# QZ1-boy/CDFO

Hardware: NVIDIA B200
Metric: HR frames/sec, 1080p x4 LD-QP37 (higher is better)
Workload: dtype bf16

## Files before the change

cdfo_b200/csrc/lra.cu:

```cuda
#include <cuda.h>
#include <cstring>

#include "cdfo_common.cuh"
#include "sm100_ptx.cuh"

namespace cdfo {

__device__ __forceinline__ float warp_max(float v) {
#pragma unroll
  for (int o = 16; o > 0; o >>= 1) v = fmaxf(v, __shfl_xor_sync(0xffffffffu, v, o));
  return v;
}
__device__ __forceinline__ float warp_sum(float v) {
#pragma unroll
  for (int o = 16; o > 0; o >>= 1) v += __shfl_xor_sync(0xffffffffu, v, o);
  return v;
}

__global__ void lra_mask_kernel(const float *__restrict__ u, const float *__restrict__ vmax, const float *__restrict__ qv,
                                uint8_t *__restrict__ midx, float *__restrict__ qsel, int HW) {
  __shared__ float vm[64];
  const int b = blockIdx.y;
  if (threadIdx.x < 64) vm[threadIdx.x] = vmax[b * 64 + threadIdx.x];
  __syncthreads();
  const int p = blockIdx.x * blockDim.x + threadIdx.x;
  if (p >= HW) return;
  const float *up = u + (size_t)b * 64 * HW + p;
  float lmax = -INFINITY, second_sum = 0.f;
  int cmax = 0;
  float l[64];
#pragma unroll
  for (int c = 0; c < 64; ++c) {
    const float g = -logf(-logf(up[(size_t)c * HW]));
    l[c] = vm[c] + g;
    if (l[c] > lmax) { lmax = l[c]; cmax = c; }
  }
#pragma unroll
  for (int c = 0; c < 64; ++c) second_sum += expf(l[c] - lmax);
  const bool on = (1.0f / second_sum) >= 0.5f;
  midx[(size_t)b * HW + p] = on ? (uint8_t)cmax : (uint8_t)255;
  qsel[(size_t)b * HW + p] = on ? qv[((size_t)b * 128 + cmax) * HW + p] : 0.f;
}

constexpr int kLd = 68;
__device__ __forceinline__ uint32_t to_tf32(float x) {
  uint32_t r;
  asm("cvt.rna.tf32.f32 %0, %1;" : "=r"(r) : "f"(x));
  return r;
}
__device__ __forceinline__ void mma_tf32(float (&d)[4], const uint32_t (&a)[4], uint32_t b0, uint32_t b1) {
  asm volatile("mma.sync.aligned.m16n8k8.row.col.f32.tf32.tf32.f32 {%0, %1, %2, %3}, {%4, %5, %6, %7}, {%8, %9}, {%0, %1, %2, %3};"
               : "+f"(d[0]), "+f"(d[1]), "+f"(d[2]), "+f"(d[3])
               : "r"(a[0]), "r"(a[1]), "r"(a[2]), "r"(a[3]), "r"(b0), "r"(b1));
}


__device__ __forceinline__ void flash_tile_block(float (&sc)[8][4], float (&m_run)[2], float (&l_run)[2], float (&o)[8][4],
                                                 const uint32_t *__restrict__ Vu, int key0, int n_keys, int g, int tq) {
  float mx[2] = {-INFINITY, -INFINITY};
#pragma unroll
  for (int n = 0; n < 8; ++n) {
    const int key = key0 + 8 * n + 2 * tq;
    if (key >= n_keys) { sc[n][0] = -INFINITY; sc[n][2] = -INFINITY; }
    if (key + 1 >= n_keys) { sc[n][1] = -INFINITY; sc[n][3] = -INFINITY; }
    mx[0] = fmaxf(mx[0], fmaxf(sc[n][0], sc[n][1]));
    mx[1] = fmaxf(mx[1], fmaxf(sc[n][2], sc[n][3]));
  }
  float scale[2];
#pragma unroll
  for (int r = 0; r < 2; ++r) {
    mx[r] = fmaxf(mx[r], __shfl_xor_sync(0xffffffffu, mx[r], 1));
    mx[r] = fmaxf(mx[r], __shfl_xor_sync(0xffffffffu, mx[r], 2));
    const float m_new = fmaxf(m_run[r], mx[r]);
    scale[r] = expf(m_run[r] - m_new);
    m_run[r] = m_new;
    l_run[r] *= scale[r];
  }
#pragma unroll
  for (int n = 0; n < 8; ++n) {
    sc[n][0] = expf(sc[n][0] - m_run[0]); sc[n][1] = expf(sc[n][1] - m_run[0]);
    sc[n][2] = expf(sc[n][2] - m_run[1]); sc[n][3] = expf(sc[n][3] - m_run[1]);
    l_run[0] += sc[n][0] + sc[n][1];
    l_run[1] += sc[n][2] + sc[n][3];
    o[n][0] *= scale[0]; o[n][1] *= scale[0]; o[n][2] *= scale[1]; o[n][3] *= scale[1];
  }
#pragma unroll
  for (int s = 0; s < 8; ++s) {
    const uint32_t ap[4] = {to_tf32(sc[s][0]), to_tf32(sc[s][2]), to_tf32(sc[s][1]), to_tf32(sc[s][3])};
    const uint32_t *vr = Vu + (key0 + 8 * s + 2 * tq) * kLd + g;
#pragma unroll
    for (int n = 0; n < 8; ++n) mma_tf32(o[n], ap, vr[8 * n], vr[kLd + 8 * n]);
  }
}

constexpr int kRowWarps = 9, kRowThreads = kRowWarps * 32;
constexpr int kRowPiece = 64;
constexpr int kRowRawBytes = 2 * 64 * kRowPiece * 4 + 64;
template <bool TMA>
__global__ void __launch_bounds__(kRowThreads, 1) lra_row_kernel(const __grid_constant__ CUtensorMap qvmap, const float *__restrict__ qv,
                                                                const uint8_t *__restrict__ midx, const float *__restrict__ qsel,
                                                                float *__restrict__ vrow_t, LraTables t, int H, int W) {
  extern __shared__ __align__(1024) float sm_all[];
  float *sm = TMA ? sm_all + kRowRawBytes / 4 : sm_all;
  const int b = blockIdx.y, h = blockIdx.x;
  const int HW = H * W;
  const int Wk = (W + 63) & ~63;
  float *vr = sm;
  float *Rs = vr + Wk * kLd;
  float *sw = Rs + 4096;
  float *e0 = sw + Wk;
  float *qs = e0 + Wk;
  float *n0 = qs + Wk;
  float *red = n0 + 64;
  int *cs = reinterpret_cast<int *>(red + kRowThreads);
  int *mlist = cs + Wk;
  __shared__ int mcount;
  __shared__ float m0_s, d0_s;
  const int tid = threadIdx.x, lane = tid & 31, warp = tid >> 5, g = lane >> 2, tq = lane & 3;
  float kw[9];
#pragma unroll
  for (int i = 0; i < 9; ++i) kw[i] = t.kw[i];
  for (int e = tid; e < 4096; e += kRowThreads) Rs[e] = t.r[e];

  if (TMA) {
    float *raw = sm_all;
    uint64_t *bars = reinterpret_cast<uint64_t *>(sm_all + 2 * 64 * kRowPiece);
    const uint32_t bar0 = ptx::smem_u32(bars);
    if (tid == 0) {
      ptx::mbar_init(bar0, 1);
      ptx::mbar_init(bar0 + 8, 1);
      ptx::mbar_init(bar0 + 16, 8);
      ptx::mbar_init(bar0 + 24, 8);
      ptx::fence_mbar_init();
    }
    __syncthreads();
    const int n_pieces = Wk / kRowPiece;
    if (warp == 8) {
      if (lane == 0) {
        for (int pc = 0; pc < n_pieces; ++pc) {
          const int st = pc & 1;
          ptx::mbar_wait_parked(bar0 + 16 + 8 * st, ((pc >> 1) & 1) ^ 1);
          ptx::mbar_arrive_expect_tx(bar0 + 8 * st, 64 * kRowPiece * 4);
          ptx::tma_load_3d(ptx::smem_u32(raw) + st * 64 * kRowPiece * 4, &qvmap, bar0 + 8 * st, pc * kRowPiece, h, b * 128 + 64);
        }
      }
    } else {
      const int px = tid & 63, c0 = (tid >> 6) * 16;
      for (int pc = 0; pc < n_pieces; ++pc) {
        const int st = pc & 1, w = pc * kRowPiece + px;
        ptx::mbar_wait_parked(bar0 + 8 * st, (pc >> 1) & 1);
        const float *rp = raw + st * 64 * kRowPiece + px;
        float win[24];
#pragma unroll
        for (int i = 0; i < 24; ++i) {
          const int c = c0 - 4 + i;
          win[i] = (c >= 0 && c < 64) ? rp[c * kRowPiece] : 0.f;
        }
        __syncwarp();
        if (lane == 0) ptx::mbar_arrive(bar0 + 16 + 8 * st);
        float *row = vr + w * kLd + c0;
#pragma unroll
        for (int c4 = 0; c4 < 4; ++c4) {
          float o[4];
#pragma unroll
          for (int j = 0; j < 4; ++j) {
            float acc = t.beta;
#pragma unroll
            for (int i = 0; i < 9; ++i) acc = fmaf(kw[i], win[4 * c4 + j + i], acc);
            o[j] = w < W ? acc : 0.f;
          }
          *reinterpret_cast<float4 *>(row + 4 * c4) = make_float4(o[0], o[1], o[2], o[3]);
        }
      }
    }
  } else {
  const float *vbase = qv + ((size_t)b * 128 + 64) * HW + (size_t)h * W;
  for (int e = tid; e < 64 * Wk; e += kRowThreads) {
    const int c = e / Wk, w = e - c * Wk;
    const bool ok = w < W;
// ... 14 lines not shown
    for (int c4 = 0; c4 < 16; ++c4) {
      const float4 v = *reinterpret_cast<const float4 *>(row + 4 * c4);
      win[4 + 4 * c4] = v.x; win[5 + 4 * c4] = v.y; win[6 + 4 * c4] = v.z; win[7 + 4 * c4] = v.w;
    }
#pragma unroll
    for (int c4 = 0; c4 < 16; ++c4) {
      float o[4];
#pragma unroll
      for (int j = 0; j < 4; ++j) {
        float acc = t.beta;
#pragma unroll
        for (int i = 0; i < 9; ++i) acc = fmaf(kw[i], win[4 * c4 + j + i], acc);
        o[j] = acc;
      }
      *reinterpret_cast<float4 *>(row + 4 * c4) = make_float4(o[0], o[1], o[2], o[3]);
    }
  }
  }
  if (tid == 0) mcount = 0;
  __syncthreads();
  for (int w = tid; w < Wk; w += kRowThreads) {
    int c = 255;
    float q = 0.f;
    if (w < W) {
      c = midx[(size_t)b * HW + h * W + w];
      q = qsel[(size_t)b * HW + h * W + w];
    }
    const bool on = c != 255;
    cs[w] = on ? c : -1;
    qs[w] = q;
    sw[w] = on ? t.beta * q * t.k1[c] : 0.f;
    if (on) mlist[atomicAdd(&mcount, 1)] = w;
  }
  __syncthreads();
  float m = -INFINITY;
  for (int w = tid; w < W; w += kRowThreads) m = fmaxf(m, sw[w]);
  m = warp_max(m);
  if (lane == 0) red[warp] = m;
  __syncthreads();
  if (tid == 0) {
    float mm = red[0];
    for (int i = 1; i < kRowWarps; ++i) mm = fmaxf(mm, red[i]);
    m0_s = mm;
  }
  __syncthreads();
  const float m0 = m0_s;
  float d = 0.f;
  for (int w = tid; w < W; w += kRowThreads) {
    const float e = expf(sw[w] - m0);
    e0[w] = e;
    d += e;
  }
  d = warp_sum(d);
  __syncthreads();
  if (lane == 0) red[warp] = d;
  __syncthreads();
  if (tid == 0) {
    float dd = 0.f;
    for (int i = 0; i < kRowWarps; ++i) dd += red[i];
    d0_s = dd;
  }
  {
    const int c = tid & 63, part = tid >> 6;
    float acc = 0.f;
    if (part < 4)
      for (int w = part; w < W; w += 4) acc = fmaf(e0[w], vr[w * kLd + c], acc);
    __syncthreads();
    red[tid] = acc;
    __syncthreads();
    if (tid < 64) n0[tid] = (red[tid] + red[tid + 64] + red[tid + 128] + red[tid + 192]) / d0_s;
  }
  __syncthreads();
  for (int e = tid; e < W * 64; e += kRowThreads) {
    const int w = e >> 6, c = e & 63;
    if (cs[w] < 0) vrow_t[(((size_t)b * W + w) * H + h) * 64 + c] = n0[c];
  }
  for (int e = tid; e < Wk * 64; e += kRowThreads) {
    float *p = vr + (e >> 6) * kLd + (e & 63);
    *p = __uint_as_float(to_tf32(*p));
  }
  __syncthreads();
  const int nm = mcount;
  const uint32_t *Vu = reinterpret_cast<const uint32_t *>(vr);
  for (int q0 = warp * 16; q0 < nm; q0 += kRowWarps * 16) {
    int wq[2], c1[2];
    float q1[2];
#pragma unroll
    for (int r = 0; r < 2; ++r) {
      const int qi = q0 + g + 8 * r;
      wq[r] = qi < nm ? mlist[qi] : -1;
      c1[r] = wq[r] >= 0 ? cs[wq[r]] : 0;
      q1[r] = wq[r] >= 0 ? qs[wq[r]] : 0.f;
    }
    float o[8][4];
#pragma unroll
    for (int n = 0; n < 8; ++n)
#pragma unroll
      for (int i = 0; i < 4; ++i) o[n][i] = 0.f;
    float m_run[2] = {-INFINITY, -INFINITY}, l_run[2] = {0.f, 0.f};
    for (int key0 = 0; key0 < Wk; key0 += 64) {
      float sc[8][4];
#pragma unroll
      for (int n = 0; n < 8; ++n) {
        const int k = key0 + 8 * n + 2 * tq;
        const float2 s2 = *reinterpret_cast<const float2 *>(sw + k), q2 = *reinterpret_cast<const float2 *>(qs + k);
        const int2 c2 = *reinterpret_cast<const int2 *>(cs + k);
#pragma unroll
        for (int r = 0; r < 2; ++r) {
          sc[n][2 * r] = c2.x >= 0 ? fmaf(q1[r] * q2.x, Rs[c1[r] * 64 + c2.x], s2.x) : s2.x;
          sc[n][2 * r + 1] = c2.y >= 0 ? fmaf(q1[r] * q2.y, Rs[c1[r] * 64 + c2.y], s2.y) : s2.y;
        }
      }
      flash_tile_block(sc, m_run, l_run, o, Vu, key0, W, g, tq);
    }
#pragma unroll
    for (int r = 0; r < 2; ++r) {
      l_run[r] += __shfl_xor_sync(0xffffffffu, l_run[r], 1);
      l_run[r] += __shfl_xor_sync(0xffffffffu, l_run[r], 2);
    }
#pragma unroll
    for (int r = 0; r < 2; ++r) {
      if (wq[r] < 0) continue;
      const float inv = 1.f / l_run[r];
      float *dst = vrow_t + (((size_t)b * W + wq[r]) * H + h) * 64 + 2 * tq;
#pragma unroll
      for (int n = 0; n < 8; ++n) *reinterpret_cast<float2 *>(dst + 8 * n) = make_float2(o[n][2 * r] * inv, o[n][2 * r + 1] * inv);
    }
  }
}


template <typename LoadKV, typename Store>
__device__ __forceinline__ void flash_block_fp32_kptr(const float *Qs, const float *const *Kptr, const float *Vs, float *Ps,
                                                      int n_keys, LoadKV key_chunk, Store store) {
  const int tid = threadIdx.x, ty = tid >> 4, tx = tid & 15;
  float m_run[4], l_run[4], o[4][4];
#pragma unroll
  for (int i = 0; i < 4; ++i) {
    m_run[i] = -INFINITY;
    l_run[i] = 0.f;
#pragma unroll
    for (int c = 0; c < 4; ++c) o[i][c] = 0.f;
  }
  const int n_chunks = (n_keys + 63) >> 6;
  for (int kb = 0; kb < n_chunks; ++kb) {
    key_chunk(kb);
    const float *Ks = *Kptr;
    float sacc[4][4];
#pragma unroll
    for (int i = 0; i < 4; ++i)
#pragma unroll
      for (int j = 0; j < 4; ++j) sacc[i][j] = 0.f;
#pragma unroll 4
    for (int k = 0; k < 64; k += 4) {
      float4 a[4], bq[4];
#pragma unroll
      for (int i = 0; i < 4; ++i) a[i] = *reinterpret_cast<const float4 *>(Qs + (ty + 16 * i) * kLd + k);
#pragma unroll
      for (int j = 0; j < 4; ++j) bq[j] = *reinterpret_cast<const float4 *>(Ks + (tx + 16 * j) * kLd + k);
#pragma unroll
      for (int i = 0; i < 4; ++i)
#pragma unroll
        for (int j = 0; j < 4; ++j) {
          sacc[i][j] = fmaf(a[i].x, bq[j].x, sacc[i][j]);
          sacc[i][j] = fmaf(a[i].y, bq[j].y, sacc[i][j]);
          sacc[i][j] = fmaf(a[i].z, bq[j].z, sacc[i][j]);
          sacc[i][j] = fmaf(a[i].w, bq[j].w, sacc[i][j]);
        }
    }
#pragma unroll
    for (int i = 0; i < 4; ++i) {
      float mx = -INFINITY;
#pragma unroll
      for (int j = 0; j < 4; ++j) {
        if (kb * 64 + tx + 16 * j >= n_keys) sacc[i][j] = -INFINITY;
        mx = fmaxf(mx, sacc[i][j]);
      }
#pragma unroll
      for (int off = 8; off > 0; off >>= 1) mx = fmaxf(mx, __shfl_xor_sync(0xffffffffu, mx, off));
      const float m_new = fmaxf(m_run[i], mx);
      const float scale = expf(m_run[i] - m_new);
      m_run[i] = m_new;
      float ps = 0.f;
#pragma unroll
      for (int j = 0; j < 4; ++j) {
        const float pv = expf(sacc[i][j] - m_new);
        Ps[(ty + 16 * i) * kLd + tx + 16 * j] = pv;
        ps += pv;
      }
      l_run[i] = l_run[i] * scale + ps;
#pragma unroll
      for (int c = 0; c < 4; ++c) o[i][c] *= scale;
    }
    __syncthreads();
#pragma unroll 4
    for (int j = 0; j < 64; j += 4) {
      float4 pr[4], vv[4];
#pragma unroll
      for (int i = 0; i < 4; ++i) pr[i] = *reinterpret_cast<const float4 *>(Ps + (ty + 16 * i) * kLd + j);
#pragma unroll
      for (int jj = 0; jj < 4; ++jj) vv[jj] = *reinterpret_cast<const float4 *>(Vs + (j + jj) * kLd + 4 * tx);
#pragma unroll
      for (int i = 0; i < 4; ++i) {
        const float pe[4] = {pr[i].x, pr[i].y, pr[i].z, pr[i].w};
#pragma unroll
        for (int jj = 0; jj < 4; ++jj) {
          o[i][0] = fmaf(pe[jj], vv[jj].x, o[i][0]);
          o[i][1] = fmaf(pe[jj], vv[jj].y, o[i][1]);
          o[i][2] = fmaf(pe[jj], vv[jj].z, o[i][2]);
// ... 367 lines not shown
    }
  }
  float mx[2] = {-INFINITY, -INFINITY}, sum[2] = {0.f, 0.f};
#pragma unroll
  for (int n = 0; n < 8; ++n) {
    mx[0] = fmaxf(mx[0], fmaxf(sc[n][0], sc[n][1]));
    mx[1] = fmaxf(mx[1], fmaxf(sc[n][2], sc[n][3]));
  }
#pragma unroll
  for (int r = 0; r < 2; ++r) {
    mx[r] = fmaxf(mx[r], __shfl_xor_sync(0xffffffffu, mx[r], 1));
    mx[r] = fmaxf(mx[r], __shfl_xor_sync(0xffffffffu, mx[r], 2));
  }
#pragma unroll
  for (int n = 0; n < 8; ++n) {
    sc[n][0] = expf(sc[n][0] - mx[0]); sc[n][1] = expf(sc[n][1] - mx[0]);
    sc[n][2] = expf(sc[n][2] - mx[1]); sc[n][3] = expf(sc[n][3] - mx[1]);
    sum[0] += sc[n][0] + sc[n][1];
    sum[1] += sc[n][2] + sc[n][3];
  }
  float o[8][4];
#pragma unroll
  for (int n = 0; n < 8; ++n)
#pragma unroll
    for (int i = 0; i < 4; ++i) o[n][i] = 0.f;
#pragma unroll
  for (int s = 0; s < 4; ++s) {
    uint32_t ap[4], apl[4];
#pragma unroll
    for (int i = 0; i < 4; ++i) {
      const float p0 = sc[2 * s + (i >> 1)][2 * (i & 1)], p1 = sc[2 * s + (i >> 1)][2 * (i & 1) + 1];
      const float h0 = __bfloat162float(__float2bfloat16_rn(p0)), h1 = __bfloat162float(__float2bfloat16_rn(p1));
      ap[i] = pack_bf16x2(h0, h1);
      apl[i] = pack_bf16x2(p0 - h0, p1 - h1);
    }
    const uint32_t *vr = Vt + g * kWinLd + 8 * s + tq, *vl = Vl + g * kWinLd + 8 * s + tq;
#pragma unroll
    for (int n = 0; n < 8; ++n) {
      const uint32_t b0 = vr[8 * n * kWinLd], b1 = vr[8 * n * kWinLd + 4];
      mma_bf16(o[n], apl, b0, b1);
      mma_bf16(o[n], ap, vl[8 * n * kWinLd], vl[8 * n * kWinLd + 4]);
      mma_bf16(o[n], ap, b0, b1);
    }
  }
#pragma unroll
  for (int r = 0; r < 2; ++r) {
    sum[r] += __shfl_xor_sync(0xffffffffu, sum[r], 1);
    sum[r] += __shfl_xor_sync(0xffffffffu, sum[r], 2);
  }
  const float inv0 = 1.f / sum[0], inv1 = 1.f / sum[1];
  const int t0 = q0r + g, t1 = t0 + 8;
  float *d0 = loc_out + (((size_t)b * H + wy * 8 + (t0 >> 3)) * W + wx * 8 + (t0 & 7)) * 64 + 2 * tq;
  float *d1 = loc_out + (((size_t)b * H + wy * 8 + (t1 >> 3)) * W + wx * 8 + (t1 & 7)) * 64 + 2 * tq;
#pragma unroll
  for (int n = 0; n < 8; ++n) {
    *reinterpret_cast<float2 *>(d0 + 8 * n) = make_float2(o[n][0] * inv0, o[n][1] * inv0);
    *reinterpret_cast<float2 *>(d1 + 8 * n) = make_float2(o[n][2] * inv1, o[n][3] * inv1);
  }
}

}

using namespace cdfo;

typedef CUresult (*LraEncodeTiledFn)(CUtensorMap *, CUtensorMapDataType, cuuint32_t, void *, const cuuint64_t *, const cuuint64_t *,
                                     const cuuint32_t *, const cuuint32_t *, CUtensorMapInterleave, CUtensorMapSwizzle,
                                     CUtensorMapL2promotion, CUtensorMapFloatOOBfill);
static LraEncodeTiledFn lra_encode_tiled_fn() {
  static LraEncodeTiledFn fn = nullptr;
  if (!fn) {
    void *ptr = nullptr;
    cudaDriverEntryPointQueryResult q;
    if (cudaGetDriverEntryPoint("cuTensorMapEncodeTiled", &ptr, cudaEnableDefault, &q) == cudaSuccess && q == cudaDriverEntryPointSuccess)
      fn = reinterpret_cast<LraEncodeTiledFn>(ptr);
  }
  return fn;
}

static bool g_lra_row_tma = true;
extern "C" int cdfo_lra_set_row_tma(int on) {
  g_lra_row_tma = on != 0;
  return CDFO_OK;
}
static bool g_lra_col_tf32 = false;
static bool g_lra_col_tc = true;
static bool g_lra_win_tc = true;
extern "C" int cdfo_lra_set_col_precision(int tf32) {
  g_lra_col_tf32 = tf32 != 0;
  return CDFO_OK;
}
extern "C" int cdfo_lra_set_col_tcgen05(int on) {
  g_lra_col_tc = on != 0;
  return CDFO_OK;
}
extern "C" int cdfo_lra_set_win_tensor_core(int on) {
  g_lra_win_tc = on != 0;
  return CDFO_OK;
}

extern "C" size_t cdfo_lra_workspace_bytes(int B, int H, int W) {
  const size_t P = (size_t)B * H * W;
  return P * (1 + 4) + 3 * P * 64 * 4 + 256;
}

static int lra_run(const float *qv, const float *u, const float *vmax, const float *x, const float *x2, const float *tables,
                   float beta, float bh, const float *fuse_w, const float *fuse_b, float *out, void *out_c8, int out_channels,
                   int channel0, void *workspace, int B, int H, int W, void *stream);

extern "C" int cdfo_lra_fwd(const float *qv, const float *u, const float *vmax, const float *x, const float *x2, const float *tables,
                            float beta, float bh, const float *fuse_w, const float *fuse_b, float *out, void *workspace, int B,
                            int H, int W, void *stream) {
  return lra_run(qv, u, vmax, x, x2, tables, beta, bh, fuse_w, fuse_b, out, nullptr, 0, 0, workspace, B, H, W, stream);
}

extern "C" int cdfo_lra_c8_fwd(const float *qv, const float *u, const float *vmax, const float *x, const float *x2, const float *tables,
                               float beta, float bh, const float *fuse_w, const float *fuse_b, void *out_c8, int out_channels,
                               int channel0, void *workspace, int B, int H, int W, void *stream) {
  CDFO_REQUIRE(out_c8 && ((uintptr_t)out_c8 & 15) == 0, CDFO_ERR_NULL, "cdfo_lra_c8_fwd: out_c8 must be a 16-byte aligned pointer");
  CDFO_REQUIRE(out_channels % 8 == 0 && channel0 % 8 == 0 && channel0 >= 0 && channel0 + 64 <= out_channels, CDFO_ERR_SHAPE,
               "cdfo_lra_c8_fwd: channels [%d, %d) do not fit %d output channels (multiples of 8)", channel0, channel0 + 64, out_channels);
  return lra_run(qv, u, vmax, x, x2, tables, beta, bh, fuse_w, fuse_b, nullptr, out_c8, out_channels, channel0, workspace, B, H, W, stream);
}

static int lra_run(const float *qv, const float *u, const float *vmax, const float *x, const float *x2, const float *tables,
                   float beta, float bh, const float *fuse_w, const float *fuse_b, float *out, void *out_c8, int out_channels,
                   int channel0, void *workspace, int B, int H, int W, void *stream) {
  CDFO_REQUIRE(qv && u && vmax && x && tables && fuse_w && fuse_b && (out || out_c8) && workspace, CDFO_ERR_NULL, "cdfo_lra_fwd: NULL pointer");
  CDFO_REQUIRE(B > 0 && B <= 65535 && H > 0 && W > 0 && H % 8 == 0 && W % 8 == 0, CDFO_ERR_SHAPE,
               "cdfo_lra_fwd: H and W must be multiples of the window size 8 (got %d x %d)", H, W);
  cudaStream_t s = (cudaStream_t)stream;
  const size_t P = (size_t)B * H * W;
  const int HW = H * W;
  uint8_t *ws = (uint8_t *)workspace;
  float *qsel = (float *)ws;
  float *vrow_t = qsel + P;
  float *long_out = vrow_t + P * 64;
  float *loc_out = long_out + P * 64;
  uint8_t *midx = (uint8_t *)(loc_out + P * 64);
  LraTables t{tables, tables + 9, tables + 18, tables + 82, beta, bh};

  lra_mask_kernel<<<dim3(ceil_div(HW, 128), B), 128, 0, s>>>(u, vmax, qv, midx, qsel, HW);

  const int Wk = (W + 63) & ~63;
  const size_t row_smem = ((size_t)Wk * kLd + 4096 + 3 * (size_t)Wk + 64 + kRowThreads + 2 * (size_t)Wk) * 4;
  const int Hk = (H + 63) & ~63;
  const size_t col_v = (size_t)Hk * kLd > (size_t)(H + 8) * 64 ? (size_t)Hk * kLd : (size_t)(H + 8) * 64;
  const size_t col_smem = ((size_t)Hk * kLd + col_v) * 4;
  const size_t win_smem = (size_t)3 * 64 * kLd * 4;
  const int kDynMax = 224 * 1024;
  CDFO_REQUIRE(row_smem <= (size_t)kDynMax && col_smem <= (size_t)kDynMax, CDFO_ERR_UNSUPPORTED,
               "cdfo_lra_fwd: frame %d x %d exceeds the shared-memory row/column buffers (W <= 704, H <= 384)", H, W);
  static bool attr = false;
  if (!attr) {
    cudaError_t e1 = cudaFuncSetAttribute(lra_row_kernel<false>, cudaFuncAttributeMaxDynamicSharedMemorySize, kDynMax);
    if (e1 == cudaSuccess) e1 = cudaFuncSetAttribute(lra_row_kernel<true>, cudaFuncAttributeMaxDynamicSharedMemorySize, kDynMax);
    cudaError_t e2 = cudaFuncSetAttribute(lra_col_kernel, cudaFuncAttributeMaxDynamicSharedMemorySize, kDynMax);
    if (e2 == cudaSuccess) e2 = cudaFuncSetAttribute(lra_col_bf16_kernel, cudaFuncAttributeMaxDynamicSharedMemorySize, kDynMax);
    cudaError_t e3 = cudaFuncSetAttribute(lra_win_kernel, cudaFuncAttributeMaxDynamicSharedMemorySize, (int)win_smem);
    if (e1 != cudaSuccess || e2 != cudaSuccess || e3 != cudaSuccess)
      return fail(CDFO_ERR_CUDA, "cdfo_lra_fwd: cudaFuncSetAttribute failed: %s", cudaGetErrorString(e1 != cudaSuccess ? e1 : (e2 != cudaSuccess ? e2 : e3)));
    attr = true;
  }
  {
    CUtensorMap qm;
    memset(&qm, 0, sizeof(qm));
    bool row_tma = g_lra_row_tma && W % 4 == 0 && ((uintptr_t)qv & 15) == 0 && row_smem + kRowRawBytes <= (size_t)kDynMax;
    if (row_tma) {
      static LraEncodeTiledFn enc = lra_encode_tiled_fn();
      if (enc) {
        const cuuint64_t gdim[3] = {(cuuint64_t)W, (cuuint64_t)H, (cuuint64_t)B * 128};
        const cuuint64_t gstr[2] = {(cuuint64_t)W * 4, (cuuint64_t)H * W * 4};
        const cuuint32_t box[3] = {kRowPiece, 1, 64};
        const cuuint32_t estr[3] = {1, 1, 1};
        CUresult cr = enc(&qm, CU_TENSOR_MAP_DATA_TYPE_FLOAT32, 3, const_cast<float *>(qv), gdim, gstr, box, estr, CU_TENSOR_MAP_INTERLEAVE_NONE,
                          CU_TENSOR_MAP_SWIZZLE_NONE, CU_TENSOR_MAP_L2_PROMOTION_L2_128B, CU_TENSOR_MAP_FLOAT_OOB_FILL_NONE);
        CDFO_REQUIRE(cr == CUDA_SUCCESS, CDFO_ERR_CUDA, "cuTensorMapEncodeTiled(qv rows) failed with CUresult %d", (int)cr);
      } else {
        row_tma = false;
      }
    }
    if (row_tma) lra_row_kernel<true><<<dim3(H, B), kRowThreads, row_smem + kRowRawBytes, s>>>(qm, qv, midx, qsel, vrow_t, t, H, W);
    else lra_row_kernel<false><<<dim3(H, B), kRowThreads, row_smem, s>>>(qm, qv, midx, qsel, vrow_t, t, H, W);
  }
  int col_done = 0;
  if (!g_lra_col_tf32 && g_lra_col_tc) {
    col_done = lra_col_sm100_launch(vrow_t, midx, qsel, long_out, t, B, H, W, s);
    if (col_done < 0) return col_done;
  }
  if (col_done) {
  } else if (g_lra_col_tf32) {
    lra_col_kernel<<<dim3(W, B), kColThreads, col_smem, s>>>(vrow_t, midx, qsel, long_out, t, H, W);
  } else {
    const size_t col16_smem = ((size_t)Hk * kQw + 64 * ((size_t)Hk / 2 + 4) + 2 * (size_t)(H + 8) + 16) * 4;
    lra_col_bf16_kernel<<<dim3(W, B), kColThreads, col16_smem, s>>>(vrow_t, midx, qsel, long_out, t, H, W);
  }
  if (g_lra_win_tc) lra_win_tc_kernel<<<dim3(W / 8, H / 8, B), kWinTcThreads, 0, s>>>(qv, midx, loc_out, H, W);
  else lra_win_kernel<<<dim3(W / 8, H / 8, B), kWinThreads, win_smem, s>>>(qv, midx, loc_out, H, W);
  if (int rc = check_launch("cdfo_lra_fwd")) return rc;
  return pointwise_conv(long_out, loc_out, fuse_w, fuse_b, x, x2, out, B, 128, 64, HW, 0, 1, s, out_c8, out_channels, channel0);
}
```

include/cdfo_b200.h:

```cpp
#ifndef CDFO_B200_H_
#define CDFO_B200_H_

#include <stddef.h>
#include <stdint.h>

#ifdef __cplusplus
extern "C" {
#endif

typedef enum cdfo_status {
  CDFO_OK = 0,
  CDFO_ERR_SHAPE = -1,
  CDFO_ERR_NULL = -2,
  CDFO_ERR_CUDA = -3,
  CDFO_ERR_UNSUPPORTED = -4,
  CDFO_ERR_NO_DEVICE = -5
} cdfo_status;

typedef enum cdfo_dtype { CDFO_F32 = 0, CDFO_F16 = 1, CDFO_BF16 = 2 } cdfo_dtype;
#define CDFO_FIELDS_F16X4 16

const char *cdfo_last_error(void);
int cdfo_version(void);
int cdfo_device_ok(int dev);
// ... 2 lines not shown
                 const void *bias, void *y, int B, int C, int H, int W, int Co, int kh, int kw,
                 int stride_h, int stride_w, int pad_h, int pad_w, int dil_h, int dil_w,
                 int groups, int dg, int dtype, void *stream);

int cdfo_dcn_sample_index(const float *offset, int32_t *idx, int B, int H, int W, int kh, int kw,
                          int stride_h, int stride_w, int pad_h, int pad_w, int dil_h, int dil_w,
                          int dg, void *stream);

int cdfo_flow_warp_fwd(const float *x, const float *flow, float *y, int B, int C, int H, int W,
                       int32_t *idx, void *stream);

int cdfo_mv2mvs(const void *mv, int mv_is_int32, float *flows, int H, int W, void *stream);
int cdfo_mv2mvs_ra(const void *mv_l0, const void *mv_l1, int mv_is_int32, float *flows, int H, int W, void *stream);
int cdfo_mv_end_fix(float *flows, int B, int H, int W, int i, int max_idx, void *stream);

int cdfo_prior_conv_fwd(const float *x, const float *w, const float *bias, float *y, int B, int Co, int H, int W, void *stream);
int cdfo_prior_conv_act_fwd(const float *x, const float *w, const float *bias, float *y, int B, int Co, int H, int W, int relu, void *stream);

int cdfo_pack_c8(const float *x_nchw, void *x_c8, int B, int C, int H, int W, void *stream);
int cdfo_pack_c8_into(const float *x_nchw, void *x_c8, int B, int C, int H, int W, int out_channels, int channel0, void *stream);
int cdfo_unpack_c8(const void *x_c8, float *x_nchw, int B, int C, int H, int W, void *stream);

int cdfo_dcn_sm100_fwd(const void *x_q4p, const void *offset, const void *mask, const float *mv,
                       const void *wpk, const float *bias, void *y, int B, int H, int W, int dg,
                       int off_dtype, int out_mode, int num_ctas, int x_batch, long long off_bstride,
                       long long msk_bstride, void *stream);
int cdfo_dcn_sm100_pack_weight(const float *w, void *wpk, void *stream);
int cdfo_pack_q4p(const float *x_nchw, void *x_q4p, int B, int C, int H, int W, void *stream);
int cdfo_dcn_tex_sm100_fwd(const void *x_q4t, const void *fields, const float *mv, const void *wpk, const float *bias,
                           void *y, int B, int H, int W, int dg, int out_mode, int num_ctas, int x_batch,
                           long long fields_bstride, void *stream);
int cdfo_dcn_tex_sm100_set_fields_path(int use_tma);
int cdfo_dcn_tex_sm100_stacked_fwd(const void *x_q4t, const void *fields, const float *mv, const void *wpk, const float *bias,
                                   void *y_stack, int n_seq, int n_groups, int stack_chunks, const int *group_chunk, int H,
                                   int W, int dg, int x_batch, void *stream);
int cdfo_dcn_tex_sm100_pack_weight(const float *w, void *wpk, void *stream);
int cdfo_mv_head_dcn_fused_sm100_fwd(const void *z_c8, const void *head_wpk, const float *head_bias, float magnitude,
                                     const void *x_q4t, const float *mv, const void *dcn_wpk, const float *dcn_bias, void *y,
                                     void *fields_out, int B, int H, int W, int out_mode, int x_batch, int num_ctas, void *stream);
int cdfo_mv_head_dcn_fused_sm100_stacked_fwd(const void *z_c8, const void *head_wpk, const float *head_bias, float magnitude,
                                             const void *x_q4t, const float *mv, const void *dcn_wpk, const float *dcn_bias,
                                             void *y_stack, int n_seq, int n_groups, int stack_chunks, const int *group_chunk,
                                             int H, int W, int x_batch, void *stream);
int cdfo_pack_q4t(const float *x_nchw, void *x_q4t, int B, int C, int H, int W, void *stream);
int cdfo_q4t_pitch(int W);
size_t cdfo_q4t_bytes(int B, int C, int H, int W);
int cdfo_conv3x3_sm100_fwd(const void *x_c8, const void *wpk, const float *bias, const void *resid_c8, void *y,
                           int B, int Cin, int Cout, int H, int W, int act, int out_mode, void *stream);
int cdfo_mv_offset_head_sm100_fwd(const void *z_c8, const void *wpk, const float *bias, const void *first, void *out,
                                  int B, int Cin, int dg, int H, int W, float magnitude, void *stream);
int cdfo_mv_offset_head_dual_sm100_fwd(const void *z_c8, const void *wpk, const float *bias, void *out, int B, int Cin, int dg, int H,
                                       int W, float magnitude, void *stream);
int cdfo_conv_last_skip_sm100_fwd(const void *x_c8, const void *wpk, const float *bias, const float *lr, float *y, int B,
                                  int Cin, int H, int W, void *stream);
int cdfo_conv3x3_sm100_pack_weight(const float *w, void *wpk, int Cout, int Cin, void *stream);
int cdfo_conv_sm100_fwd(const void *x_c8, const void *wpk, const float *bias, const void *resid_c8, void *y, int B, int Cin,
                        int Cout, int H, int W, int ksize, int act, int out_mode, void *stream);
int cdfo_conv_sm100_pack_weight(const float *w, void *wpk, int Cout, int Cin, int ksize, void *stream);
size_t cdfo_conv_sm100_weight_bytes(int Cout, int Cin, int ksize);
size_t cdfo_conv3x3_sm100_weight_bytes(int Cout, int Cin);
int cdfo_conv3x3_sm100_ntile(int Cout, int Cin);
int cdfo_mdta_fwd(const float *x, int x_batch, const float *extra, const float *pred, const float *flow,
                  const float *fusion_w, const float *du_w1, const float *du_b1, const float *du_w2, const float *du_b2,
                  const float *temperature, const float *proj_w, int heads, int mode, void *out, float *ca_sums,
                  void *workspace, int B, int H, int W, void *stream);
int cdfo_mdta_c8_fwd(const void *x_c8, int x_batch, const void *extra_c8, const void *pred_c8, const float *flow, const float *fusion_w,
                     const float *du_w1, const float *du_b1, const float *du_w2, const float *du_b2, const float *temperature,
                     const float *proj_w, int heads, void *out_c8, void *workspace, int B, int H, int W, void *stream);
size_t cdfo_mdta_workspace_bytes(int B, int H, int W, int heads);
int cdfo_mdta_parts(int B);
int cdfo_channel_gate_fwd(const float *partial_sums, int parts, const float *w1, const float *b1, const float *w2,
                          const float *b2, float *gate, int B, int C, int Cmid, int HW, void *stream);
int cdfo_pack_c8_scaled(const float *x_nchw, const float *scale, void *x_c8, int B, int C, int H, int W, void *stream);
int cdfo_unpack_c8_add(const void *x_c8, const float *add_nchw, int add_batch, float *y_nchw, int B, int C, int H, int W,
                       void *stream);
int cdfo_resample_c8(const void *a, const void *b, const void *base, void *y, int B, int C, int Ho, int Wo, int mode, void *stream);
int cdfo_lra_fwd(const float *qv, const float *u, const float *vmax, const float *x, const float *x2, const float *tables,
                 float beta, float bh, const float *fuse_w, const float *fuse_b, float *out, void *workspace, int B, int H, int W,
                 void *stream);
int cdfo_lra_set_col_precision(int tf32);
int cdfo_lra_set_col_tcgen05(int on);
int cdfo_lra_set_win_tensor_core(int on);
int cdfo_lra_set_row_tma(int on);
int cdfo_lra_c8_fwd(const float *qv, const float *u, const float *vmax, const float *x, const float *x2, const float *tables,
                    float beta, float bh, const float *fuse_w, const float *fuse_b, void *out_c8, int out_channels, int channel0,
                    void *workspace, int B, int H, int W, void *stream);
int cdfo_pointwise_conv_fwd(const float *in1, const float *in2, const float *w, const float *bias, const float *resid1,
                            const float *resid2, float *out, int B, int K, int Co, int H, int W, int act, int mode, void *stream);
int cdfo_pointwise_conv_c8_fwd(const float *in1, const float *in2, const float *w, const float *bias, const float *resid1,
                               const float *resid2, void *out_c8, int B, int K, int Co, int H, int W, int act, int mode,
                               int out_channels, int channel0, void *stream);
size_t cdfo_lra_workspace_bytes(int B, int H, int W);
int cdfo_layernorm_c_fwd(const void *x, const float *gamma, const float *beta, void *y, int B, int C, int H, int W, float eps,
                         int dtype, void *stream);
int cdfo_dwconv3x3_fwd(const void *x, const float *w, void *y, int B, int C, int H, int W, int dtype, void *stream);
int cdfo_mdta_gram_fwd(const void *qk, float *partial, int B, int Ctot, int H, int W, int parts, int dtype, void *stream);
int cdfo_conv3x3_pair_sm100_supported(int Cout, int Cin);
size_t cdfo_conv3x3_pair_sm100_weight_bytes(int Cout, int Cin);
int cdfo_conv3x3_pair_sm100_pack_weight(const float *w, void *wpk, int Cout, int Cin, void *stream);
int cdfo_conv3x3_pair_sm100_fwd(const void *x_c8, const void *wpk, const float *bias, const void *resid_c8, void *y_c8, int B, int Cin,
                                int Cout, int H, int W, int act, void *stream);
int cdfo_conv3x3_pair_sm100_planes_fwd(const void *x_c8, const void *wpk, const float *bias, const void *resid_c8, void *y, int B,
                                       int Cin, int Cout, int H, int W, int act, int y_planes, void *stream);
int cdfo_conv3x3_pair_sm100_edge_fwd(const void *x_c8, const void *wpk, const float *bias, const float *bias_edge, const void *resid_c8,
                                     void *y, int B, int Cin, int Cout, int H, int W, int act, int y_planes, void *stream);
int cdfo_conv3x3_pair_sm100_up2_fwd(const void *x8_1x, const void *wpk, const float *bias, const float *bias_edge, void *y, int B, int Cin,
                                    int Cout, int H2, int W2, int act, int y_planes, void *stream);
int cdfo_conv4x4s2_pair_sm100_supported(int Cout, int Cin);
size_t cdfo_conv4x4s2_pair_sm100_weight_bytes(int Cin);
int cdfo_conv4x4s2_pair_sm100_pack_weight(const float *w3, void *wpk, int Cin, void *stream);
int cdfo_conv4x4s2_pair_sm100_fwd(const void *x_c8, const void *wpk, const float *bias, const void *resid_c8, void *y_c8, int B, int Cin,
                                  int H_in, int W_in, void *stream);
int cdfo_conv4x4s2_pair_sm100_planes_fwd(const void *x, const void *wpk, const float *bias, const void *resid_c8, void *y_c8, int B,
                                         int Cin, int H_in, int W_in, int x_planes, void *stream);
int cdfo_conv4x4s2_pair_sm100_block_fwd(const void *x, const void *wpk, const float *bias, const void *resid_c8, const void *up_c8,
                                        void *y_c8, void *half_c8, int B, int Cin, int H_in, int W_in, int x_planes, void *stream);
int cdfo_planes_to_unit_f32(const void *src, int src_kind, float *dst, int n_planes, int H_in, int W, int H_out, void *stream);
int cdfo_sr_to_u8(const float *sr, uint8_t *out, int n_planes, int H_in, int W, int H_out, void *stream);
size_t cdfo_psnr_ssim_workspace_bytes(int B, int H, int W, int border);
int cdfo_psnr_ssim_u8(const uint8_t *res, const uint8_t *gt, int B, int H, int W, int border, double *frame_out, double *accum,
                      void *workspace, void *stream);
int cdfo_umma_selftest(const void *A, const void *B, float *D, int swap_lbo_sbo, void *stream);

size_t cdfo_lra_mask_logits_workspace_bytes(int B, int H, int W);
int cdfo_lra_mask_logits_fwd(const float *v, const float *w2, const float *b2, const float *w3, const float *b3, float *vmax,
                             void *workspace, int B, int H, int W, void *stream);
int cdfo_lra_set_logit_tma(int on);

int cdfo_prior_conv_c8_fwd(const float *x, const float *w, const float *bias, void *y_c8, int B, int Co, int H, int W, int lrelu, void *stream);
int cdfo_layernorm_c8_fwd(const void *x_c8, const float *gamma, const float *beta, void *y_c8, int B, int H, int W, float eps, void *stream);
int cdfo_dwconv3x3_c8_fwd(const void *x_c8, const float *w, void *y_c8, int B, int C, int H, int W, void *stream);
int cdfo_mdta_gram_c8_fwd(const void *qkv_c8, float *partial, int B, int C, int H, int W, int parts, void *stream);
int cdfo_mdta_fold_fwd(const float *partial, const float *temperature, const float *project_out, float *M, int B, int parts, void *stream);
int cdfo_mdta_apply_c8_fwd(const void *qkv_c8, int C, int v_channel0, const float *M, const void *x1_c8, const void *x2_c8, void *out1_c8,
                           void *out2_c8, int B, int H, int W, void *stream);
int cdfo_conv16_c8_fwd(const void *x_c8, const float *w, const float *bias, void *y_c8, int B, int Hi, int Wi, int Ho, int Wo, int y_channels,
                       int transposed, void *stream);
int cdfo_spatial_gate_c8_fwd(const void *x_c8, const float *w, const float *bias, void *pooled_ws, void *y_c8, int B, int H, int W, void *stream);

#ifdef __cplusplus
}
#endif
#endif
```

Measured before the change: 89.58.

## Add persistent warp-specialized LRA row kernel with TMA pipeline and dynamic tile scheduling

Replaces the one-block-per-row LRA row kernel with a persistent kernel of SM-count blocks. A producer warp streams qv pieces through a multi-stage mbarrier/TMA ring, and consumer warps build the window rows and prefetch the next row's mask and qsel with cp.async. Masked query tiles are handed out through a shared atomic counter to balance work across warps. The aim is to hide load latency and cut launch and tail costs, at the price of more shared memory and more complex synchronisation.

```diff
diff --git a/cdfo_b200/csrc/lra.cu b/cdfo_b200/csrc/lra.cu
--- a/cdfo_b200/csrc/lra.cu
+++ b/cdfo_b200/csrc/lra.cu
@@ -95,6 +95,55 @@
 
 constexpr int kRowWarps = 9, kRowThreads = kRowWarps * 32;
 constexpr int kRowPiece = 64;
+
+__device__ __forceinline__ void row_masked_tile(int q0, int nm, const int *mlist, const int *cs, const float *qs, const float *sw,
+                                                const float *Rs, const uint32_t *Vu, float *__restrict__ vrow_t, int b, int h, int H,
+                                                int W, int Wk, int g, int tq) {
+  int wq[2], c1[2];
+  float q1[2];
+#pragma unroll
+  for (int r = 0; r < 2; ++r) {
+    const int qi = q0 + g + 8 * r;
+    wq[r] = qi < nm ? mlist[qi] : -1;
+    c1[r] = wq[r] >= 0 ? cs[wq[r]] : 0;
+    q1[r] = wq[r] >= 0 ? qs[wq[r]] : 0.f;
+  }
+  float o[8][4];
+#pragma unroll
+  for (int n = 0; n < 8; ++n)
+#pragma unroll
+    for (int i = 0; i < 4; ++i) o[n][i] = 0.f;
+  float m_run[2] = {-INFINITY, -INFINITY}, l_run[2] = {0.f, 0.f};
+  for (int key0 = 0; key0 < Wk; key0 += 64) {
+    float sc[8][4];
+#pragma unroll
+    for (int n = 0; n < 8; ++n) {
+      const int k = key0 + 8 * n + 2 * tq;
+      const float2 s2 = *reinterpret_cast<const float2 *>(sw + k), q2 = *reinterpret_cast<const float2 *>(qs + k);
+      const int2 c2 = *reinterpret_cast<const int2 *>(cs + k);
+#pragma unroll
+      for (int r = 0; r < 2; ++r) {
+        sc[n][2 * r] = c2.x >= 0 ? fmaf(q1[r] * q2.x, Rs[c1[r] * 64 + c2.x], s2.x) : s2.x;
+        sc[n][2 * r + 1] = c2.y >= 0 ? fmaf(q1[r] * q2.y, Rs[c1[r] * 64 + c2.y], s2.y) : s2.y;
+      }
+    }
+    flash_tile_block(sc, m_run, l_run, o, Vu, key0, W, g, tq);
+  }
+#pragma unroll
+  for (int r = 0; r < 2; ++r) {
+    l_run[r] += __shfl_xor_sync(0xffffffffu, l_run[r], 1);
+    l_run[r] += __shfl_xor_sync(0xffffffffu, l_run[r], 2);
+  }
+#pragma unroll
+  for (int r = 0; r < 2; ++r) {
+    if (wq[r] < 0) continue;
+    const float inv = 1.f / l_run[r];
+    float *dst = vrow_t + (((size_t)b * W + wq[r]) * H + h) * 64 + 2 * tq;
+#pragma unroll
+    for (int n = 0; n < 8; ++n) *reinterpret_cast<float2 *>(dst + 8 * n) = make_float2(o[n][2 * r] * inv, o[n][2 * r + 1] * inv);
+  }
+}
+
 constexpr int kRowRawBytes = 2 * 64 * kRowPiece * 4 + 64;
 template <bool TMA>
 __global__ void __launch_bounds__(kRowThreads, 1) lra_row_kernel(const __grid_constant__ CUtensorMap qvmap, const float *__restrict__ qv,
@@ -275,49 +324,194 @@
   __syncthreads();
   const int nm = mcount;
   const uint32_t *Vu = reinterpret_cast<const uint32_t *>(vr);
-  for (int q0 = warp * 16; q0 < nm; q0 += kRowWarps * 16) {
-    int wq[2], c1[2];
-    float q1[2];
-#pragma unroll
-    for (int r = 0; r < 2; ++r) {
-      const int qi = q0 + g + 8 * r;
-      wq[r] = qi < nm ? mlist[qi] : -1;
-      c1[r] = wq[r] >= 0 ? cs[wq[r]] : 0;
-      q1[r] = wq[r] >= 0 ? qs[wq[r]] : 0.f;
-    }
-    float o[8][4];
-#pragma unroll
-    for (int n = 0; n < 8; ++n)
-#pragma unroll
-      for (int i = 0; i < 4; ++i) o[n][i] = 0.f;
-    float m_run[2] = {-INFINITY, -INFINITY}, l_run[2] = {0.f, 0.f};
-    for (int key0 = 0; key0 < Wk; key0 += 64) {
-      float sc[8][4];
-#pragma unroll
-      for (int n = 0; n < 8; ++n) {
-        const int k = key0 + 8 * n + 2 * tq;
-        const float2 s2 = *reinterpret_cast<const float2 *>(sw + k), q2 = *reinterpret_cast<const float2 *>(qs + k);
-        const int2 c2 = *reinterpret_cast<const int2 *>(cs + k);
-#pragma unroll
-        for (int r = 0; r < 2; ++r) {
-          sc[n][2 * r] = c2.x >= 0 ? fmaf(q1[r] * q2.x, Rs[c1[r] * 64 + c2.x], s2.x) : s2.x;
-          sc[n][2 * r + 1] = c2.y >= 0 ? fmaf(q1[r] * q2.y, Rs[c1[r] * 64 + c2.y], s2.y) : s2.y;
+  for (int q0 = warp * 16; q0 < nm; q0 += kRowWarps * 16) row_masked_tile(q0, nm, mlist, cs, qs, sw, Rs, Vu, vrow_t, b, h, H, W, Wk, g, tq);
+}
+
+constexpr int kRowN0Warps = 2;
+__device__ __forceinline__ void named_bar_sync(int id, int n) { asm volatile("bar.sync %0, %1;" ::"r"(id), "r"(n) : "memory"); }
+__device__ __forceinline__ void cp_async4(void *dst, const void *src) {
+  asm volatile("cp.async.ca.shared.global [%0], [%1], 4;" ::"r"((uint32_t)__cvta_generic_to_shared(dst)), "l"(src) : "memory");
+}
+__host__ __device__ constexpr size_t row_persistent_smem(int Wk, int n_stages) {
+  return (size_t)n_stages * 64 * kRowPiece * 4 + 128 + ((size_t)Wk * kLd + 4096 + 3 * (size_t)Wk + 64 + 32 + 256 + 3 * (size_t)Wk + Wk / 4) * 4;
+}
+
+__global__ void __launch_bounds__(kRowThreads, 1) lra_row_persistent_kernel(const __grid_constant__ CUtensorMap qvmap, const uint8_t *__restrict__ midx,
+                                                                           const float *__restrict__ qsel, float *__restrict__ vrow_t, LraTables t,
+                                                                           int B, int H, int W, int n_stages) {
+  extern __shared__ __align__(1024) float sm_all[];
+  const int Wk = (W + 63) & ~63;
+  const int HW = H * W, n_rows = B * H, n_pieces = Wk / kRowPiece;
+  float *raw = sm_all;
+  uint64_t *bars = reinterpret_cast<uint64_t *>(raw + n_stages * 64 * kRowPiece);
+  float *vr = reinterpret_cast<float *>(bars + 16);
+  float *Rs = vr + Wk * kLd;
+  float *sw = Rs + 4096;
+  float *e0 = sw + Wk;
+  float *qs = e0 + Wk;
+  float *n0 = qs + Wk;
+  float *red = n0 + 64;
+  float *n0part = red + 32;
+  int *cs = reinterpret_cast<int *>(n0part + 256);
+  int *mlist = cs + Wk;
+  float *qstage = reinterpret_cast<float *>(mlist + Wk);
+  uint8_t *mstage = reinterpret_cast<uint8_t *>(qstage + Wk);
+  __shared__ int mcount[2], tiles_taken[2];
+  const int tid = threadIdx.x, lane = tid & 31, warp = tid >> 5, g = lane >> 2, tq = lane & 3;
+  const uint32_t bar0 = ptx::smem_u32(bars);
+  if (tid == 0) {
+    for (int s = 0; s < n_stages; ++s) {
+      ptx::mbar_init(bar0 + 8 * s, 1);
+      ptx::mbar_init(bar0 + 8 * (n_stages + s), 8);
+    }
+    ptx::fence_mbar_init();
+    mcount[0] = mcount[1] = 0;
+    tiles_taken[0] = tiles_taken[1] = 0;
+  }
+  for (int e = tid; e < 4096; e += kRowThreads) Rs[e] = t.r[e];
+  __syncthreads();
+
+  if (warp == 8) {
+    if (lane == 0) {
+      int pcg = 0;
+      for (int r = blockIdx.x; r < n_rows; r += gridDim.x) {
+        const int b = r / H, h = r - b * H;
+        for (int pc = 0; pc < n_pieces; ++pc, ++pcg) {
+          const int st = pcg % n_stages;
+          ptx::mbar_wait_parked(bar0 + 8 * (n_stages + st), ((pcg / n_stages) & 1) ^ 1);
+          ptx::mbar_arrive_expect_tx(bar0 + 8 * st, 64 * kRowPiece * 4);
+          ptx::tma_load_3d(ptx::smem_u32(raw) + st * 64 * kRowPiece * 4, &qvmap, bar0 + 8 * st, pc * kRowPiece, h, b * 128 + 64);
         }
       }
-      flash_tile_block(sc, m_run, l_run, o, Vu, key0, W, g, tq);
-    }
-#pragma unroll
-    for (int r = 0; r < 2; ++r) {
-      l_run[r] += __shfl_xor_sync(0xffffffffu, l_run[r], 1);
-      l_run[r] += __shfl_xor_sync(0xffffffffu, l_run[r], 2);
-    }
-#pragma unroll
-    for (int r = 0; r < 2; ++r) {
-      if (wq[r] < 0) continue;
-      const float inv = 1.f / l_run[r];
-      float *dst = vrow_t + (((size_t)b * W + wq[r]) * H + h) * 64 + 2 * tq;
-#pragma unroll
-      for (int n = 0; n < 8; ++n) *reinterpret_cast<float2 *>(dst + 8 * n) = make_float2(o[n][2 * r] * inv, o[n][2 * r + 1] * inv);
+    }
+    return;
+  }
+
+  constexpr int kC = kRowThreads - 32;
+  float kw[9];
+#pragma unroll
+  for (int i = 0; i < 9; ++i) kw[i] = t.kw[i];
+  auto stage_row = [&](int r) {
+    const size_t base = (size_t)(r / H) * HW + (size_t)(r % H) * W;
+    for (int w = tid; w < W; w += kC) cp_async4(qstage + w, qsel + base + w);
+    for (int j = tid; j < W / 4; j += kC) cp_async4(mstage + 4 * j, midx + base + 4 * j);
+    asm volatile("cp.async.commit_group;" ::: "memory");
+  };
+  if (blockIdx.x < n_rows) stage_row(blockIdx.x);
+  const int px = tid & 63, c0 = (tid >> 6) * 16;
+  auto round_piece = [&](int pc) {
+    for (int e = tid; e < kRowPiece * 16; e += kC) {
+      float4 *p = reinterpret_cast<float4 *>(vr + (pc * kRowPiece + (e >> 4)) * kLd) + (e & 15);
+      float4 v = *p;
+      v.x = __uint_as_float(to_tf32(v.x)); v.y = __uint_as_float(to_tf32(v.y));
+      v.z = __uint_as_float(to_tf32(v.z)); v.w = __uint_as_float(to_tf32(v.w));
+      *p = v;
+    }
+  };
+  int pcg = 0, it = 0;
+  for (int r = blockIdx.x; r < n_rows; r += gridDim.x, ++it) {
+    const int b = r / H, h = r - b * H, par = it & 1;
+    asm volatile("cp.async.wait_all;" ::: "memory");
+    named_bar_sync(1, kC);
+    if (tid == 0) {
+      mcount[par ^ 1] = 0;
+      tiles_taken[par ^ 1] = 0;
+    }
+    float m = -INFINITY;
+    for (int w = tid; w < Wk; w += kC) {
+      int c = 255;
+      float q = 0.f;
+      if (w < W) {
+        c = mstage[w];
+        q = qstage[w];
+      }
+      const bool on = c != 255;
+      cs[w] = on ? c : -1;
+      qs[w] = q;
+      const float s = on ? t.beta * q * t.k1[c] : 0.f;
+      sw[w] = s;
+      if (w < W) m = fmaxf(m, s);
+      if (on) mlist[atomicAdd(&mcount[par], 1)] = w;
+    }
+    m = warp_max(m);
+    if (lane == 0) red[warp] = m;
+    named_bar_sync(1, kC);
+    if (r + (int)gridDim.x < n_rows) stage_row(r + gridDim.x);
+    float m0 = red[0];
+#pragma unroll
+    for (int i = 1; i < 8; ++i) m0 = fmaxf(m0, red[i]);
+    {
+      float d = 0.f, d8 = 0.f;
+      for (int w = tid; w < W; w += kRowThreads) {
+        const float e = expf(sw[w] - m0);
+        e0[w] = e;
+        d += e;
+      }
+      if (warp == 0)
+        for (int w = kC + lane; w < W; w += kRowThreads) {
+          const float e = expf(sw[w] - m0);
+          e0[w] = e;
+          d8 += e;
+        }
+      d = warp_sum(d);
+      d8 = warp_sum(d8);
+      if (lane == 0) red[8 + warp] = d;
+      if (tid == 0) red[16] = d8;
+    }
+    float nacc = 0.f;
+    for (int pc = 0; pc < n_pieces; ++pc, ++pcg) {
+      const int st = pcg % n_stages, w = pc * kRowPiece + px;
+      ptx::mbar_wait_parked(bar0 + 8 * st, (pcg / n_stages) & 1);
+      const float *rp = raw + st * 64 * kRowPiece + px;
+      float win[24];
+#pragma unroll
+      for (int i = 0; i < 24; ++i) {
+        const int c = c0 - 4 + i;
+        win[i] = (c >= 0 && c < 64) ? rp[c * kRowPiece] : 0.f;
+      }
+      __syncwarp();
+      if (lane == 0) ptx::mbar_arrive(bar0 + 8 * (n_stages + st));
+      float *row = vr + w * kLd + c0;
+#pragma unroll
+      for (int c4 = 0; c4 < 4; ++c4) {
+        float o[4];
+#pragma unroll
+        for (int j = 0; j < 4; ++j) {
+          float acc = t.beta;
+#pragma unroll
+          for (int i = 0; i < 9; ++i) acc = fmaf(kw[i], win[4 * c4 + j + i], acc);
+          o[j] = w < W ? acc : 0.f;
+        }
+        *reinterpret_cast<float4 *>(row + 4 * c4) = make_float4(o[0], o[1], o[2], o[3]);
+      }
+      named_bar_sync(1, kC);
+      const int w_end = min(W, (pc + 1) * kRowPiece);
+      for (int w = pc * kRowPiece + (tid >> 6); w < w_end; w += 4) nacc = fmaf(e0[w], vr[w * kLd + (tid & 63)], nacc);
+      if (pc > 0) round_piece(pc - 1);
+    }
+    n0part[tid] = nacc;
+    named_bar_sync(1, kC);
+    round_piece(n_pieces - 1);
+    named_bar_sync(1, kC);
+    float d0 = 0.f;
+#pragma unroll
+    for (int i = 0; i < kRowWarps; ++i) d0 += red[8 + i];
+    const int nm = mcount[par], n_tiles = (nm + 15) >> 4;
+    if (warp < kRowN0Warps) {
+      n0[tid] = (n0part[tid] + n0part[tid + 64] + n0part[tid + 128] + n0part[tid + 192]) / d0;
+      named_bar_sync(2, kRowN0Warps * 32);
+      const float4 v = reinterpret_cast<const float4 *>(n0)[tid & 15];
+      float *dst = vrow_t + ((size_t)b * W * H + h) * 64 + 4 * (tid & 15);
+      for (int w = tid >> 4; w < W; w += kRowN0Warps * 2)
+        if (cs[w] < 0) *reinterpret_cast<float4 *>(dst + (size_t)w * H * 64) = v;
+    }
+    const uint32_t *Vu = reinterpret_cast<const uint32_t *>(vr);
+    for (;;) {
+      int tile = 0;
+      if (lane == 0) tile = atomicAdd(&tiles_taken[par], 1);
+      tile = __shfl_sync(0xffffffffu, tile, 0);
+      if (tile >= n_tiles) break;
+      row_masked_tile(tile * 16, nm, mlist, cs, qs, sw, Rs, Vu, vrow_t, b, h, H, W, Wk, g, tq);
     }
   }
 }
@@ -851,6 +1045,11 @@
   g_lra_row_tma = on != 0;
   return CDFO_OK;
 }
+static bool g_lra_row_persistent = true;
+extern "C" int cdfo_lra_set_row_persistent(int on) {
+  g_lra_row_persistent = on != 0;
+  return CDFO_OK;
+}
 static bool g_lra_col_tf32 = false;
 static bool g_lra_col_tc = true;
 static bool g_lra_win_tc = true;
@@ -923,6 +1122,7 @@
   if (!attr) {
     cudaError_t e1 = cudaFuncSetAttribute(lra_row_kernel<false>, cudaFuncAttributeMaxDynamicSharedMemorySize, kDynMax);
     if (e1 == cudaSuccess) e1 = cudaFuncSetAttribute(lra_row_kernel<true>, cudaFuncAttributeMaxDynamicSharedMemorySize, kDynMax);
+    if (e1 == cudaSuccess) e1 = cudaFuncSetAttribute(lra_row_persistent_kernel, cudaFuncAttributeMaxDynamicSharedMemorySize, kDynMax);
     cudaError_t e2 = cudaFuncSetAttribute(lra_col_kernel, cudaFuncAttributeMaxDynamicSharedMemorySize, kDynMax);
     if (e2 == cudaSuccess) e2 = cudaFuncSetAttribute(lra_col_bf16_kernel, cudaFuncAttributeMaxDynamicSharedMemorySize, kDynMax);
     cudaError_t e3 = cudaFuncSetAttribute(lra_win_kernel, cudaFuncAttributeMaxDynamicSharedMemorySize, (int)win_smem);
@@ -948,7 +1148,18 @@
         row_tma = false;
       }
     }
-    if (row_tma) lra_row_kernel<true><<<dim3(H, B), kRowThreads, row_smem + kRowRawBytes, s>>>(qm, qv, midx, qsel, vrow_t, t, H, W);
+    const int row_stages = row_persistent_smem(Wk, 3) <= (size_t)kDynMax ? 3 : 2;
+    if (row_tma && g_lra_row_persistent && row_persistent_smem(Wk, row_stages) <= (size_t)kDynMax) {
+      static int n_sm = 0;
+      if (!n_sm) {
+        int dev = 0;
+        cudaError_t e = cudaGetDevice(&dev);
+        if (e == cudaSuccess) e = cudaDeviceGetAttribute(&n_sm, cudaDevAttrMultiProcessorCount, dev);
+        CDFO_REQUIRE(e == cudaSuccess && n_sm > 0, CDFO_ERR_CUDA, "cdfo_lra_fwd: SM count query failed: %s", cudaGetErrorString(e));
+      }
+      const int grid = B * H < n_sm ? B * H : n_sm;
+      lra_row_persistent_kernel<<<grid, kRowThreads, row_persistent_smem(Wk, row_stages), s>>>(qm, midx, qsel, vrow_t, t, B, H, W, row_stages);
+    } else if (row_tma) lra_row_kernel<true><<<dim3(H, B), kRowThreads, row_smem + kRowRawBytes, s>>>(qm, qv, midx, qsel, vrow_t, t, H, W);
     else lra_row_kernel<false><<<dim3(H, B), kRowThreads, row_smem, s>>>(qm, qv, midx, qsel, vrow_t, t, H, W);
   }
   int col_done = 0;
diff --git a/include/cdfo_b200.h b/include/cdfo_b200.h
--- a/include/cdfo_b200.h
+++ b/include/cdfo_b200.h
@@ -108,6 +108,7 @@
 int cdfo_lra_set_col_tcgen05(int on);
 int cdfo_lra_set_win_tensor_core(int on);
 int cdfo_lra_set_row_tma(int on);
+int cdfo_lra_set_row_persistent(int on);
 int cdfo_lra_c8_fwd(const float *qv, const float *u, const float *vmax, const float *x, const float *x2, const float *tables,
                     float beta, float bh, const float *fuse_w, const float *fuse_b, void *out_c8, int out_channels, int channel0,
                     void *workspace, int B, int H, int W, void *stream);
```

Result: no change. 90.43 (median of 6 runs) (+0.9%).
